# bbuhrow/avx-ecm

Measured on AMD Instinct MI355X. Metric: stage-1 curves/sec at B1=1000000, 416-bit N, higher is better.
Workload: dtype u32 (28-bit limbs, 64-bit accumulate)

## Files before the change

### avx-ecm_amd/csrc/gecm_row.hpp

```cpp
#pragma once
#include "gecm_curve.hpp"
#include "gecm_rowk.h"

template <int NQ>
struct FeR {
    int32_t v[NQ];
};

template <int NQ>
struct RowMod {
    uint32_t n[NQ];
    uint32_t rho;
    int32_t c16;
};

__device__ __forceinline__ void row_pin(const int64_t &x)
{
    asm volatile("" ::"v"(x));
}
__device__ __forceinline__ int32_t row_c16()
{
    int32_t c;
    asm volatile("s_mov_b32 %0, 16" : "=s"(c));
    return c;
}

#define GECM_DPP_ROW_SHL1 0x101
#define GECM_DPP_ROW_SHR1 0x111
#define GECM_DPP_ROW_NEWBCAST 0x150

template <int CTRL>
__device__ __forceinline__ uint32_t row_dpp(uint32_t x)
{
    return (uint32_t)__builtin_amdgcn_update_dpp(0, (int)x, CTRL, 0xF, 0xF, true);
}
template <int I>
__device__ __forceinline__ uint32_t row_bcast(uint32_t x)
{
    return row_dpp<GECM_DPP_ROW_NEWBCAST + I>(x);
}
template <int I>
__device__ __forceinline__ int64_t row_bcast64(int64_t x)
{
    return __builtin_amdgcn_update_dpp((int64_t)0, x, GECM_DPP_ROW_NEWBCAST + I, 0xF, 0xF, true);
}
template <int I>
__device__ __forceinline__ uint32_t row_bcast_lds(uint32_t x)
{
    return (uint32_t)__builtin_amdgcn_ds_swizzle((int)x, 0x10 | (I << 5));
}
__device__ __forceinline__ uint32_t other_row(uint32_t x)
{
    return (uint32_t)__builtin_amdgcn_ds_swizzle((int)x, 0x401F );
}

__device__ __forceinline__ void smad(int64_t &acc, int32_t x, int32_t y)
{
    asm("v_mad_i64_i32 %0, vcc, %1, %2, %0" : "+v"(acc) : "v"(x), "v"(y) : "vcc");
}
__device__ __forceinline__ void umad(int64_t &acc, uint32_t x, uint32_t y)
{
    asm("v_mad_u64_u32 %0, vcc, %1, %2, %0" : "+v"(acc) : "v"(x), "v"(y) : "vcc");
}
__device__ __forceinline__ int64_t smad0(int32_t x, int32_t y)
{
    int64_t r;
    asm("v_mad_i64_i32 %0, vcc, %1, %2, 0" : "=v"(r) : "v"(x), "v"(y) : "vcc");
    return r;
}
__device__ __forceinline__ int64_t smad16(int32_t x, int64_t add)
{
    int64_t r;
    asm("v_mad_i64_i32 %0, vcc, %1, 16, %2" : "=v"(r) : "v"(x), "v"(add) : "vcc");
    return r;
}

__device__ __forceinline__ int64_t smad16_smad(int32_t x, int64_t add, int32_t y, int32_t z)
{
    int64_t r;
    asm("v_mad_i64_i32 %0, vcc, %1, 16, %2\n\tv_mad_i64_i32 %0, vcc, %3, %4, %0" : "=&v"(r) : "v"(x), "v"(add), "v"(y), "v"(z) : "vcc");
    return r;
}

template <int NQ, int ROWS, bool RHO1, bool ALDS>
__device__ __forceinline__ void fer_mul(FeR<NQ> &r, const FeR<NQ> &a, const FeR<NQ> &b, const RowMod<NQ> &m)
{
    static_assert(ROWS > 16 * (NQ - 1) && ROWS <= 16 * NQ, "the limbs in use fill the lanes but for the last one");
    static_assert(!ALDS || NQ == 1, "the crossbar form is for one limb per lane");
    int32_t a4[NQ], b4[NQ];
#pragma unroll
    for (int t = 0; t < NQ; t++) {
        a4[t] = (int32_t)((uint32_t)a.v[t] << 2);
        b4[t] = (int32_t)((uint32_t)b.v[t] << 2);
    }
    if constexpr (NQ >= 2) {
        int64_t T[NQ];
        const int64_t a01 = (int64_t)(((uint64_t)(uint32_t)a4[1] << 32) | (uint32_t)a4[0]);
        int64_t Ap = row_bcast64<0>(a01);
        int32_t As = 0;
        auto limb = [&](auto jc) -> int32_t {
            constexpr int q = decltype(jc)::value % NQ;
            return q == 0 ? (int32_t)(uint32_t)Ap : q == 1 ? (int32_t)(Ap >> 32) : As;
        };
#pragma unroll
        for (int t = 0; t < NQ; t++) T[t] = (int64_t)limb(IC<0>{}) * b4[t];
        static_for<0, ROWS>([&](auto ic) {
            constexpr int i = decltype(ic)::value;
            constexpr int rot = i % NQ, nxt = (i + 1) % NQ;
            const uint32_t Q = row_bcast<0>(RHO1 ? (uint32_t)T[rot] : (uint32_t)T[rot] * m.rho);
            __builtin_amdgcn_sched_barrier(0);
#pragma unroll
            for (int t = 0; t < NQ; t++) {
                T[(t + rot) % NQ] = (int64_t)((uint64_t)T[(t + rot) % NQ] + (uint64_t)Q * m.n[t]);
                __builtin_amdgcn_sched_barrier(0);
            }
            const int32_t Ac = limb(IC<i + 1>{});
            if constexpr (i + 1 < ROWS) {
#pragma unroll
                for (int t = 0; t < NQ - 1; t++) {
                    T[(t + nxt) % NQ] += (int64_t)Ac * b4[t];
                    row_pin(T[(t + nxt) % NQ]);
                    __builtin_amdgcn_sched_barrier(0);
                }
            }
            const int32_t hi = (int32_t)(T[rot] >> 32);
            const uint32_t lo = row_dpp<GECM_DPP_ROW_SHL1>((uint32_t)T[rot]);
            __builtin_amdgcn_sched_barrier(0);
            T[nxt] += (int64_t)hi * m.c16;
            row_pin(T[nxt]);
            __builtin_amdgcn_sched_barrier(0);
            if constexpr (i + 1 < ROWS) {
                T[rot] = (int64_t)Ac * b4[NQ - 1] + (int64_t)(uint64_t)lo;
                row_pin(T[rot]);
            } else {
                T[rot] = (int64_t)(uint64_t)lo;
            }
            __builtin_amdgcn_sched_barrier(0);
            if constexpr (i + 2 < ROWS) {
                if constexpr ((i + 2) % NQ == 0) Ap = row_bcast64<(i + 2) / NQ>(a01);
                else if constexpr ((i + 2) % NQ == 2) As = (int32_t)row_bcast<(i + 2) / NQ>((uint32_t)a4[NQ - 1]);
                __builtin_amdgcn_sched_barrier(0);
            }
        });
        int32_t lo[NQ];
        int32_t carry = 0;
#pragma unroll
        for (int t = 0; t < NQ - 1; t++) {
            int64_t u16 = T[(t + ROWS) % NQ] + (int64_t)(1u << 31);
            if (t > 0) u16 += (int64_t)carry * m.c16;
            carry = (int32_t)(u16 >> 32);
            lo[t] = (int32_t)(((uint32_t)u16 >> 4) & GECM_LIMB_MASK) - (1 << 27);
        }
        const int32_t ut = (int32_t)(T[(NQ - 1 + ROWS) % NQ] >> 4) + carry + (1 << 27);
        lo[NQ - 1] = (int32_t)((uint32_t)ut & GECM_LIMB_MASK) - (1 << 27);
        const int32_t below = (int32_t)row_dpp<GECM_DPP_ROW_SHR1>((uint32_t)(ut >> GECM_LIMB_BITS));
        r.v[0] = lo[0] + below;
#pragma unroll
        for (int t = 1; t < NQ; t++) r.v[t] = lo[t];
    } else {
        int32_t Ab[ROWS];
        int64_t a01 = 0;
        if constexpr (!ALDS) a01 = (int64_t)(((uint64_t)row_dpp<GECM_DPP_ROW_SHL1>((uint32_t)a4[0]) << 32) | (uint32_t)a4[0]);
        auto request = [&](auto jc) {
            constexpr int j = decltype(jc)::value;
            if constexpr (ALDS) {
                Ab[j] = (int32_t)row_bcast_lds<j>((uint32_t)a4[0]);
            } else if constexpr (j % 2 == 0) {
                const int64_t P = row_bcast64<j>(a01);
                Ab[j] = (int32_t)(uint32_t)P;
                if constexpr (j + 1 < ROWS) Ab[j + 1] = (int32_t)(P >> 32);
            }
        };
        if constexpr (ALDS) static_for<0, ROWS>(request);
        else request(IC<0>{});
        int64_t T[NQ];
#pragma unroll
        for (int t = 0; t < NQ; t++) T[t] = 0;
        static_for<0, ROWS>([&](auto ic) {
            constexpr int i = decltype(ic)::value;
            if constexpr (i == 0) T[0] = smad0(Ab[0], b4[0]);
            if constexpr (!ALDS) {
                __builtin_amdgcn_sched_barrier(0);
                if constexpr (i + 1 < ROWS) request(IC<i + 1>{});
                __builtin_amdgcn_sched_barrier(0);
            }
            uint32_t qs = (uint32_t)T[0];
            if (!RHO1) qs *= m.rho;
            const uint32_t Q = row_bcast<0>(qs);
            umad(T[0], Q, m.n[0]);
            if constexpr (!ALDS) __builtin_amdgcn_sched_barrier(0);
            const int32_t hi = (int32_t)(T[0] >> 32);
            const uint32_t lo = row_dpp<GECM_DPP_ROW_SHL1>((uint32_t)T[0]);
            if constexpr (i + 1 < ROWS) T[0] = smad16_smad(hi, (int64_t)(uint64_t)lo, Ab[i + 1], b4[0]);
            else T[0] = smad16(hi, (int64_t)(uint64_t)lo);
        });
        const int64_t u16 = T[0] + (int64_t)(1u << 31);
        const int32_t lim = (int32_t)(((uint32_t)u16 >> 4) & GECM_LIMB_MASK) - (1 << 27);
        r.v[0] = lim + (int32_t)row_dpp<GECM_DPP_ROW_SHR1>((uint32_t)(u16 >> 32));
    }
}

template <int NQ>
struct PtR {
    FeR<NQ> own;
    FeR<NQ> sd;
    FeR<NQ> ds;
    FeR<NQ> oth;
};

struct RowSign {
    uint32_t mz, bz;
    uint32_t mx, bx;
};

template <int NQ>
__device__ __forceinline__ void fer_other(FeR<NQ> &r, const FeR<NQ> &a)
{
#pragma unroll
    for (int t = 0; t < NQ; t++) r.v[t] = (int32_t)other_row((uint32_t)a.v[t]);
}

template <int NQ>
__device__ __forceinline__ void fer_sum_diff(FeR<NQ> &r, const FeR<NQ> &oth, const FeR<NQ> &own, const RowSign &g)
{
#pragma unroll
    for (int t = 0; t < NQ; t++) r.v[t] = (int32_t)((uint32_t)oth.v[t] + ((uint32_t)own.v[t] ^ g.mz) + g.bz);
}

template <int NQ>
__device__ __forceinline__ void row_forms(PtR<NQ> &p, const RowSign &g)
{
    fer_other<NQ>(p.oth, p.own);
    fer_sum_diff<NQ>(p.sd, p.oth, p.own, g);
#pragma unroll
    for (int t = 0; t < NQ; t++)
        p.ds.v[t] = (int32_t)((uint32_t)p.own.v[t] + ((uint32_t)p.oth.v[t] ^ g.mx) + g.bx);
}

template <int NQ, int ROWS, bool ALDS>
__device__ __forceinline__ void row_add(PtR<NQ> &T, const FeR<NQ> &fB, const FeR<NQ> &fA, const FeR<NQ> &c, bool isZ,
                                        const RowSign &g, const RowMod<NQ> &m)
{
    FeR<NQ> w, t, e;
    fer_mul<NQ, ROWS, true, ALDS>(w, fB, fA, m);
    fer_other<NQ>(t, w);
    fer_sum_diff<NQ>(e, t, w, g);
    fer_mul<NQ, ROWS, true, ALDS>(e, e, e, m);
    fer_mul<NQ, ROWS, true, ALDS>(T.own, e, c, m);
    row_forms<NQ>(T, g);
}

template <int NQ, int ROWS, bool ALDS>
__device__ __forceinline__ void row_dup(PtR<NQ> &D, const FeR<NQ> &fA, const FeR<NQ> &s4, bool isZ, const RowSign &g,
                                        const RowMod<NQ> &m)
{
    FeR<NQ> q, t, w, p1, p2, r1;
    fer_mul<NQ, ROWS, true, ALDS>(q, fA, fA, m);
    fer_other<NQ>(t, q);
#pragma unroll
    for (int i = 0; i < NQ; i++) {
        w.v[i] = t.v[i] - q.v[i];
        p1.v[i] = isZ ? s4.v[i] : q.v[i];
        p2.v[i] = isZ ? w.v[i] : t.v[i];
    }
    fer_mul<NQ, ROWS, true, ALDS>(r1, p1, p2, m);
#pragma unroll
    for (int i = 0; i < NQ; i++) t.v[i] = r1.v[i] + q.v[i];
    fer_mul<NQ, ROWS, true, ALDS>(t, t, w, m);
#pragma unroll
    for (int i = 0; i < NQ; i++) D.own.v[i] = isZ ? t.v[i] : r1.v[i];
    row_forms<NQ>(D, g);
}

template <int NQ>
__device__ __forceinline__ void fer_load(FeR<NQ> &r, const uint32_t *__restrict__ base, size_t stride, uint32_t cidx,
                                         uint32_t l, uint32_t nl)
{
#pragma unroll
    for (int t = 0; t < NQ; t++) {
        const uint32_t limb = (uint32_t)NQ * l + (uint32_t)t;
        r.v[t] = limb < nl ? (int32_t)base[(size_t)limb * stride + cidx] : 0;
    }
}

template <int NQ, int ROWS, bool ALDS>
__device__ __forceinline__ void run_tape_row(const uint32_t *__restrict__ tape, uint32_t tape_len, PtR<NQ> &A,
                                             const FeR<NQ> &s4, bool isZ, const RowSign &g, const RowMod<NQ> &m)
{
    PtR<NQ> B = A, C = A;
    auto fetch = [&](uint32_t pc) -> uint32_t {
        uint32_t w = tape[pc >> 2];
        return __builtin_amdgcn_readfirstlane((w >> ((pc & 3u) * 8u)) & 0xffu);
    };
    uint32_t nxt = tape_len ? fetch(0) : GECM_OP_NOP;
    for (uint32_t pc = 0; pc < tape_len; pc++) {
        uint32_t op = nxt;
        nxt = (pc + 1 < tape_len) ? fetch(pc + 1) : GECM_OP_NOP;
        while ((op & ~GECM_OP_SWAP) == (GECM_OP_STEP | GECM_OP_RULE3)) {
            if (op & GECM_OP_SWAP) {
                PtR<NQ> t = A;
                A = B;
                B = t;
            }
            PtR<NQ> T;
            row_add<NQ, ROWS, ALDS>(T, B.ds, A.sd, C.oth, isZ, g, m);
            C = B;
            B = T;
            pc++;
            op = nxt;
            nxt = (pc + 1 < tape_len) ? fetch(pc + 1) : GECM_OP_NOP;
        }
        if (op == GECM_OP_NOP) continue;
        const uint32_t rule = op & GECM_OP_RULE_MASK;
        const bool is_step = op >= GECM_OP_STEP;
        const bool do_add = op != GECM_OP_PRAC_BEGIN;
        const bool do_dup = op != GECM_OP_PRAC_END;
        if (is_step && (op & GECM_OP_SWAP)) {
            PtR<NQ> t = A;
            A = B;
            B = t;
        }
        if (is_step && rule == GECM_OP_RULE5) {
            PtR<NQ> t = B;
            B = C;
            C = t;
        } else if (is_step && rule == GECM_OP_RULE9) {
            PtR<NQ> t = A;
            A = B;
            B = C;
            C = t;
        } else if (op == GECM_OP_PRAC_BEGIN) {
            B = A;
            C = A;
        }
        PtR<NQ> T, D;
        if (do_add) row_add<NQ, ROWS, ALDS>(T, B.ds, A.sd, C.oth, isZ, g, m);
        if (do_dup) row_dup<NQ, ROWS, ALDS>(D, A.sd, s4, isZ, g, m);
        if (op == GECM_OP_PRAC_END) {
            A = T;
        } else if (op == GECM_OP_PRAC_BEGIN) {
            A = D;
        } else if (rule == GECM_OP_RULE4) {
            B = T;
            A = D;
        } else if (rule == GECM_OP_RULE5) {
            PtR<NQ> t = C;
            C = T;
            B = t;
            A = D;
        } else {
            PtR<NQ> oldA = C;
            C = T;
            B = D;
            A = oldA;
        }
    }
}


template <int NQ, int ROWS, bool ALDS>
__device__ __forceinline__ void stage1_row(const uint32_t *__restrict__ tape, uint32_t tape_len, uint32_t *__restrict__ X,
                                           uint32_t *__restrict__ Z, const uint32_t *__restrict__ S, size_t stride,
                                           uint32_t nl, const uint32_t *__restrict__ rc, uint32_t rho_n)
{
    const uint32_t cidx = (blockIdx.x * blockDim.x + threadIdx.x) >> 5;
    const uint32_t l = threadIdx.x & 15u;
    const bool isZ = (threadIdx.x & 16u) != 0;
    uint32_t *mine = isZ ? Z : X;
    RowMod<NQ> mp, mn;
    FeR<NQ> cin, one, kp;
#pragma unroll
    for (int t = 0; t < NQ; t++) {
        const uint32_t j = (uint32_t)NQ * l + (uint32_t)t;
        mp.n[t] = rc[0 * GECM_ROW_WORDS + j];
        mn.n[t] = rc[1 * GECM_ROW_WORDS + j];
        cin.v[t] = (int32_t)rc[2 * GECM_ROW_WORDS + j];
        one.v[t] = (int32_t)rc[3 * GECM_ROW_WORDS + j];
        kp.v[t] = (int32_t)rc[4 * GECM_ROW_WORDS + j];
    }
    mp.rho = 1u;
    mn.rho = rho_n;
    mp.c16 = mn.c16 = row_c16();
    PtR<NQ> P;
    FeR<NQ> s4, t;
    fer_load<NQ>(t, mine, stride, cidx, l, nl);
    fer_mul<NQ, ROWS, true, ALDS>(P.own, t, cin, mp);
    RowSign g;
    g.mz = isZ ? 0xffffffffu : 0u;
    g.bz = isZ ? 1u : 0u;
    g.mx = ~g.mz;
    g.bx = 1u - g.bz;
    row_forms<NQ>(P, g);
    fer_load<NQ>(t, S, stride, cidx, l, nl);
    fer_mul<NQ, ROWS, true, ALDS>(s4, t, cin, mp);
    run_tape_row<NQ, ROWS, ALDS>(tape, tape_len, P, s4, isZ, g, mp);
    fer_mul<NQ, ROWS, false, ALDS>(t, P.own, one, mn);
    uint32_t u[NQ];
#pragma unroll
    for (int i = 0; i < NQ; i++) u[i] = (uint32_t)(t.v[i] + kp.v[i]);
    const uint32_t below = row_dpp<GECM_DPP_ROW_SHR1>(u[NQ - 1] >> GECM_LIMB_BITS);
#pragma unroll
    for (int i = 0; i < NQ; i++) {
        const uint32_t limb = (uint32_t)NQ * l + (uint32_t)i;
        const uint32_t v = (u[i] & GECM_LIMB_MASK) + (i == 0 ? below : (u[i - 1] >> GECM_LIMB_BITS));
        if (limb < nl) mine[(size_t)limb * stride + cidx] = (limb == nl - 1) ? v + (u[i] & ~GECM_LIMB_MASK) : v;
    }
}
```

Baseline: 1598.

## Keep field elements pre-shifted by two bits across multiplications

```diff
diff --git a/avx-ecm_amd/csrc/gecm_row.hpp b/avx-ecm_amd/csrc/gecm_row.hpp
--- a/avx-ecm_amd/csrc/gecm_row.hpp
+++ b/avx-ecm_amd/csrc/gecm_row.hpp
@@ -18,6 +18,12 @@
 {
     asm volatile("" ::"v"(x));
 }
+__device__ __forceinline__ uint32_t row_hi(int64_t x)
+{
+    uint32_t h = (uint32_t)(x >> 32);
+    asm("" : "+v"(h));
+    return h;
+}
 __device__ __forceinline__ int32_t row_c16()
 {
     int32_t c;
@@ -90,8 +96,8 @@
     int32_t a4[NQ], b4[NQ];
 #pragma unroll
     for (int t = 0; t < NQ; t++) {
-        a4[t] = (int32_t)((uint32_t)a.v[t] << 2);
-        b4[t] = (int32_t)((uint32_t)b.v[t] << 2);
+        a4[t] = a.v[t];
+        b4[t] = b.v[t];
     }
     if constexpr (NQ >= 2) {
         int64_t T[NQ];
@@ -142,21 +148,15 @@
                 __builtin_amdgcn_sched_barrier(0);
             }
         });
-        int32_t lo[NQ];
         int32_t carry = 0;
 #pragma unroll
-        for (int t = 0; t < NQ - 1; t++) {
+        for (int t = 0; t < NQ; t++) {
             int64_t u16 = T[(t + ROWS) % NQ] + (int64_t)(1u << 31);
             if (t > 0) u16 += (int64_t)carry * m.c16;
             carry = (int32_t)(u16 >> 32);
-            lo[t] = (int32_t)(((uint32_t)u16 >> 4) & GECM_LIMB_MASK) - (1 << 27);
+            r.v[t] = (int32_t)((uint32_t)u16 + 0x80000000u) >> 2;
         }
-        const int32_t ut = (int32_t)(T[(NQ - 1 + ROWS) % NQ] >> 4) + carry + (1 << 27);
-        lo[NQ - 1] = (int32_t)((uint32_t)ut & GECM_LIMB_MASK) - (1 << 27);
-        const int32_t below = (int32_t)row_dpp<GECM_DPP_ROW_SHR1>((uint32_t)(ut >> GECM_LIMB_BITS));
-        r.v[0] = lo[0] + below;
-#pragma unroll
-        for (int t = 1; t < NQ; t++) r.v[t] = lo[t];
+        r.v[0] += (int32_t)row_dpp<GECM_DPP_ROW_SHR1>((uint32_t)carry << 2);
     } else {
         int32_t Ab[ROWS];
         int64_t a01 = 0;
@@ -195,8 +195,8 @@
             else T[0] = smad16(hi, (int64_t)(uint64_t)lo);
         });
         const int64_t u16 = T[0] + (int64_t)(1u << 31);
-        const int32_t lim = (int32_t)(((uint32_t)u16 >> 4) & GECM_LIMB_MASK) - (1 << 27);
-        r.v[0] = lim + (int32_t)row_dpp<GECM_DPP_ROW_SHR1>((uint32_t)(u16 >> 32));
+        const int32_t lim4 = (int32_t)(uint32_t)T[0] >> 2;
+        r.v[0] = lim4 + (int32_t)row_dpp<GECM_DPP_ROW_SHR1>(row_hi(u16) << 2);
     }
 }
 
@@ -384,6 +384,12 @@
     PtR<NQ> P;
     FeR<NQ> s4, t;
     fer_load<NQ>(t, mine, stride, cidx, l, nl);
+#pragma unroll
+    for (int i = 0; i < NQ; i++) {
+        cin.v[i] = (int32_t)((uint32_t)cin.v[i] << 2);
+        one.v[i] = (int32_t)((uint32_t)one.v[i] << 2);
+        t.v[i] = (int32_t)((uint32_t)t.v[i] << 2);
+    }
     fer_mul<NQ, ROWS, true, ALDS>(P.own, t, cin, mp);
     RowSign g;
     g.mz = isZ ? 0xffffffffu : 0u;
@@ -392,12 +398,14 @@
     g.bx = 1u - g.bz;
     row_forms<NQ>(P, g);
     fer_load<NQ>(t, S, stride, cidx, l, nl);
+#pragma unroll
+    for (int i = 0; i < NQ; i++) t.v[i] = (int32_t)((uint32_t)t.v[i] << 2);
     fer_mul<NQ, ROWS, true, ALDS>(s4, t, cin, mp);
     run_tape_row<NQ, ROWS, ALDS>(tape, tape_len, P, s4, isZ, g, mp);
     fer_mul<NQ, ROWS, false, ALDS>(t, P.own, one, mn);
     uint32_t u[NQ];
 #pragma unroll
-    for (int i = 0; i < NQ; i++) u[i] = (uint32_t)(t.v[i] + kp.v[i]);
+    for (int i = 0; i < NQ; i++) u[i] = (uint32_t)((t.v[i] >> 2) + kp.v[i]);
     const uint32_t below = row_dpp<GECM_DPP_ROW_SHR1>(u[NQ - 1] >> GECM_LIMB_BITS);
 #pragma unroll
     for (int i = 0; i < NQ; i++) {
```

Result: no change. 1601, median of 6 (+0.2%).
